# TimZaman/dotaclient

Hardware: NVIDIA H100
Metric: optimizer_steps_per_sec (higher is better)
Workload: dtype f32

## Files before the change

dotaclient_b200/csrc/encoder.cu:

```cuda
#include "dc_common.cuh"
#include "unit_basic.cuh"

namespace {

constexpr int kC = 128;
constexpr int kIn = kUnitFeatures;
constexpr int kWarps = 8;
constexpr int kThreadsE = kWarps * 32;
constexpr int kMaxUnits = 40;

__global__ void unit_basic_bwd_reduce_kernel(const float *__restrict__ partial, int nblocks, float *__restrict__ dw_b,
                                             float *__restrict__ db_b, int accumulate) {
    const int i = blockIdx.x * blockDim.x + threadIdx.x;
    if (i >= kC * (kIn + 1)) return;
    float s = 0.f;
    for (int b = 0; b < nblocks; ++b) s += partial[(size_t)b * kC * (kIn + 1) + i];
    const int o = i / (kIn + 1), k = i % (kIn + 1);
    float *dst = k < kIn ? dw_b + o * kIn + k : db_b + o;
    *dst = accumulate ? *dst + s : s;
}

constexpr int kEnvIn = 3;
__global__ void __launch_bounds__(kThreadsE) env_fwd_kernel(const float *__restrict__ env, const float *__restrict__ w_e,
                                                            const float *__restrict__ b_e, float *__restrict__ out, int ld,
                                                            int64_t N) {
    const int lane = threadIdx.x & 31, warp = threadIdx.x >> 5;
    float w[4][kEnvIn], b[4];
#pragma unroll
    for (int c = 0; c < 4; ++c) {
        b[c] = b_e[lane * 4 + c];
#pragma unroll
        for (int k = 0; k < kEnvIn; ++k) w[c][k] = w_e[(lane * 4 + c) * kEnvIn + k];
    }
    const int64_t rows_per_iter = (int64_t)gridDim.x * kWarps * 32;
    for (int64_t base = ((int64_t)blockIdx.x * kWarps + warp) * 32; base < N; base += rows_per_iter) {
        const int nrows = (int)min((int64_t)32, N - base);
        float e[kEnvIn];
#pragma unroll
        for (int k = 0; k < kEnvIn; ++k) e[k] = lane < nrows ? env[(base + lane) * kEnvIn + k] : 0.f;
        for (int r = 0; r < nrows; ++r) {
            float a[4] = {b[0], b[1], b[2], b[3]};
#pragma unroll
            for (int k = 0; k < kEnvIn; ++k) {
                const float u = __shfl_sync(0xffffffffu, e[k], r);
#pragma unroll
                for (int c = 0; c < 4; ++c) a[c] = fmaf(u, w[c][k], a[c]);
            }
            *reinterpret_cast<float4 *>(out + (base + r) * ld + lane * 4) =
                make_float4(fmaxf(a[0], 0.f), fmaxf(a[1], 0.f), fmaxf(a[2], 0.f), fmaxf(a[3], 0.f));
        }
    }
}

__global__ void __launch_bounds__(kThreadsE) env_bwd_kernel(const float *__restrict__ d_out, const float *__restrict__ out, int ld,
                                                            const float *__restrict__ env, int64_t N,
                                                            float *__restrict__ partial) {
    __shared__ float s_red[kC][kEnvIn + 1];
    const int lane = threadIdx.x & 31, warp = threadIdx.x >> 5;
    float acc[4][kEnvIn + 1];
#pragma unroll
    for (int c = 0; c < 4; ++c)
#pragma unroll
        for (int k = 0; k <= kEnvIn; ++k) acc[c][k] = 0.f;
    const int64_t rows_per_iter = (int64_t)gridDim.x * kWarps * 32;
    for (int64_t base = ((int64_t)blockIdx.x * kWarps + warp) * 32; base < N; base += rows_per_iter) {
        const int nrows = (int)min((int64_t)32, N - base);
        float e[kEnvIn];
#pragma unroll
        for (int k = 0; k < kEnvIn; ++k) e[k] = lane < nrows ? env[(base + lane) * kEnvIn + k] : 0.f;
        for (int r0 = 0; r0 < nrows; r0 += 8) {
            float4 g4[8], y4[8];
#pragma unroll
            for (int j = 0; j < 8; ++j) {
                const int r = min(r0 + j, nrows - 1);
                g4[j] = __ldg(reinterpret_cast<const float4 *>(d_out + (base + r) * ld) + lane);
                y4[j] = __ldg(reinterpret_cast<const float4 *>(out + (base + r) * ld) + lane);
            }
#pragma unroll
            for (int j = 0; j < 8; ++j) {
                const bool live = r0 + j < nrows;
                const float g[4] = {live && y4[j].x > 0.f ? g4[j].x : 0.f, live && y4[j].y > 0.f ? g4[j].y : 0.f,
                                    live && y4[j].z > 0.f ? g4[j].z : 0.f, live && y4[j].w > 0.f ? g4[j].w : 0.f};
#pragma unroll
                for (int k = 0; k < kEnvIn; ++k) {
                    const float u = __shfl_sync(0xffffffffu, e[k], min(r0 + j, 31));
#pragma unroll
                    for (int c = 0; c < 4; ++c) acc[c][k] = fmaf(g[c], u, acc[c][k]);
                }
#pragma unroll
                for (int c = 0; c < 4; ++c) acc[c][kEnvIn] += g[c];
            }
        }
    }
    for (int w = 0; w < kWarps; ++w) {
        if (warp == w) {
#pragma unroll
            for (int c = 0; c < 4; ++c)
#pragma unroll
                for (int k = 0; k <= kEnvIn; ++k) {
                    float *dst = &s_red[lane * 4 + c][k];
                    *dst = (w == 0 ? 0.f : *dst) + acc[c][k];
                }
        }
        __syncthreads();
    }
    for (int i = threadIdx.x; i < kC * (kEnvIn + 1); i += kThreadsE)
        partial[(size_t)blockIdx.x * kC * (kEnvIn + 1) + i] = (&s_red[0][0])[i];
}

__global__ void __launch_bounds__(256) env_bwd_reduce_kernel(const float *__restrict__ partial, int nblocks, float *__restrict__ dw_e,
                                                             float *__restrict__ db_e) {
    __shared__ float sh[8][32];
    const int x = threadIdx.x & 31, y = threadIdx.x >> 5;
    const int i = blockIdx.x * 32 + x;
    float s = 0.f;
    if (i < kC * (kEnvIn + 1))
        for (int b = y; b < nblocks; b += 8) s += partial[(size_t)b * kC * (kEnvIn + 1) + i];
    sh[y][x] = s;
    __syncthreads();
    if (y == 0 && i < kC * (kEnvIn + 1)) {
        float t = 0.f;
#pragma unroll
        for (int r = 0; r < 8; ++r) t += sh[r][x];
        const int o = i / (kEnvIn + 1), k = i % (kEnvIn + 1);
        if (k < kEnvIn) dw_e[o * kEnvIn + k] = t; else db_e[o] = t;
    }
}

struct UnitPtrs { const float *p[6]; };
__host__ __device__ constexpr int group_units(int g) { return g == 1 ? 5 : (g == 2 || g == 3) ? 16 : 1; }
__host__ __device__ constexpr int group_offset(int g) { return g == 0 ? 0 : g == 1 ? 1 : g == 2 ? 6 : g == 3 ? 22 : g == 4 ? 38 : 39; }
constexpr int kTokenU4 = kMaxUnits * kIn / 4;

__device__ __forceinline__ void load_basic_weights(float (&w)[4][kIn], float (&b)[4], const float *__restrict__ w_b,
                                                   const float *__restrict__ b_b, int lane) {
#pragma unroll
    for (int c = 0; c < 4; ++c) {
        b[c] = __ldg(b_b + 4 * lane + c);
#pragma unroll
        for (int k = 0; k < kIn; ++k) w[c][k] = __ldg(w_b + (4 * lane + c) * kIn + k);
    }
}

__device__ __forceinline__ void stage_token_units(float4 *su, const UnitPtrs &units, int64_t n, int lane) {
#pragma unroll
    for (int g = 0; g < 6; ++g) {
        const int cnt = 3 * group_units(g);
        const float4 *src = reinterpret_cast<const float4 *>(units.p[g]) + n * cnt;
        for (int j = lane; j < cnt; j += 32) su[3 * group_offset(g) + j] = __ldg(src + j);
    }
}

__device__ __forceinline__ float4 basic_row(const float4 *row, const float (&w)[4][kIn], const float (&b)[4]) {
    const float4 u0 = row[0], u1 = row[1], u2 = row[2];
    const float u[kIn] = {u0.x, u0.y, u0.z, u0.w, u1.x, u1.y, u1.z, u1.w, u2.x, u2.y, u2.z, u2.w};
    return make_float4(dc_unit_basic(u, w[0], b[0]), dc_unit_basic(u, w[1], b[1]), dc_unit_basic(u, w[2], b[2]),
                       dc_unit_basic(u, w[3], b[3]));
}

__global__ void __launch_bounds__(kThreadsE) target_unit_q_fwd_kernel(const float *__restrict__ q, int ld_q, UnitPtrs units,
                                                                      const float *__restrict__ w_b, const float *__restrict__ b_b,
                                                                      float *__restrict__ logits, int64_t N) {
    __shared__ float4 s_u[kWarps][kTokenU4];
    const int lane = threadIdx.x & 31, warp = threadIdx.x >> 5;
    float w[4][kIn], b[4];
    load_basic_weights(w, b, w_b, b_b, lane);
    float4 *su = s_u[warp];
    for (int64_t n = (int64_t)blockIdx.x * kWarps + warp; n < N; n += (int64_t)gridDim.x * kWarps) {
        const float *qrow = q + n * ld_q;
        __syncwarp();
        stage_token_units(su, units, n, lane);
        __syncwarp();
        float mine = 0.f, mine_hi = 0.f;
#pragma unroll
        for (int g = 0; g < 6; ++g) {
            const float4 a = __ldg(reinterpret_cast<const float4 *>(qrow + g * kC) + lane);
            const float c = __ldg(qrow + 6 * kC + g);
            const int nu = group_units(g), off = group_offset(g);
            for (int u = 0; u < nu; ++u) {
                const float4 v = basic_row(su + 3 * (off + u), w, b);
                float d = v.x * a.x + v.y * a.y + v.z * a.z + v.w * a.w;
                d = dc_warp_sum(d) + c;
                const int o = off + u;
                if (o < 32) { if (lane == o) mine = d; } else { if (lane == o - 32) mine_hi = d; }
            }
        }
        logits[n * kMaxUnits + lane] = mine;
        if (lane < kMaxUnits - 32) logits[n * kMaxUnits + 32 + lane] = mine_hi;
    }
}

__global__ void __launch_bounds__(kThreadsE) target_unit_q_bwd_kernel(const float *__restrict__ dlogits, UnitPtrs units,
                                                                      const float *__restrict__ w_b, const float *__restrict__ b_b,
                                                                      float *__restrict__ s, int ld_s, int64_t N) {
    __shared__ float4 s_u[kWarps][kTokenU4];
    const int lane = threadIdx.x & 31, warp = threadIdx.x >> 5;
    float w[4][kIn], b[4];
    load_basic_weights(w, b, w_b, b_b, lane);
    float4 *su = s_u[warp];
    const float4 zero = make_float4(0.f, 0.f, 0.f, 0.f);
    for (int64_t n = (int64_t)blockIdx.x * kWarps + warp; n < N; n += (int64_t)gridDim.x * kWarps) {
        const float g_lo = dlogits[n * kMaxUnits + lane];
        const float g_hi = lane < kMaxUnits - 32 ? dlogits[n * kMaxUnits + 32 + lane] : 0.f;
        const bool any = __any_sync(0xffffffffu, g_lo != 0.f || g_hi != 0.f);
        float4 *srow = reinterpret_cast<float4 *>(s + n * ld_s) + lane;
        if (!any) {
#pragma unroll
            for (int g = 0; g < 7; ++g) srow[g * (kC / 4)] = zero;
            continue;
        }
        __syncwarp();
        stage_token_units(su, units, n, lane);
        __syncwarp();
        float sig[6];
#pragma unroll
        for (int g = 0; g < 6; ++g) {
            const int nu = group_units(g), off = group_offset(g);
            float4 acc = zero;
            float sg = 0.f;
            for (int u = 0; u < nu; ++u) {
                const int o = off + u;
                const float gv = __shfl_sync(0xffffffffu, o < 32 ? g_lo : g_hi, o & 31);
                const float4 v = basic_row(su + 3 * o, w, b);
                acc.x = fmaf(gv, v.x, acc.x); acc.y = fmaf(gv, v.y, acc.y); acc.z = fmaf(gv, v.z, acc.z); acc.w = fmaf(gv, v.w, acc.w);
                sg += gv;
            }
            srow[g * (kC / 4)] = acc;
            sig[g] = sg;
        }
        float4 tail = zero;
        if (lane == 0) tail = make_float4(sig[0], sig[1], sig[2], sig[3]);
        if (lane == 1) tail = make_float4(sig[4], sig[5], 0.f, 0.f);
        srow[6 * (kC / 4)] = tail;
    }
}

static unsigned head_grid(int per_sm, int64_t N) {
    const int64_t want = (N + kWarps - 1) / kWarps, cap = (int64_t)(per_sm < 1 ? 1 : per_sm) * dc_sm_count();
    return (unsigned)(want < cap ? want : cap);
}

static int unit_ptrs(const float *const units[6], UnitPtrs *up, const char *who) {
    DC_REQUIRE(units != nullptr, DC_EINVAL, "%s: units is NULL", who);
    for (int g = 0; g < 6; ++g) {
        DC_REQUIRE(units[g] && ((uintptr_t)units[g] & 15) == 0, DC_EINVAL, "%s: units[%d] null / not 16-byte aligned", who, g);
        up->p[g] = units[g];
    }
    return DC_OK;
}

}

extern "C" size_t dc_unit_basic_bwd_workspace_bytes(void) { return (size_t)4 * 1024 * kC * (kIn + 1) * sizeof(float); }

int dc_unit_basic_reduce(const float *partial, int nblocks, float *dw_b, float *db_b, int accumulate, cudaStream_t st) {
    unit_basic_bwd_reduce_kernel<<<(kC * (kIn + 1) + 255) / 256, 256, 0, st>>>(partial, nblocks, dw_b, db_b, accumulate);
    DC_LAUNCH_OK();
    return DC_OK;
}

extern "C" int dc_env_fwd(const float *env, const float *w_e, const float *b_e, float *out, int ld_out, int64_t N,
                          dc_stream_t stream) {
    DC_REQUIRE(env && w_e && b_e && out && N > 0 && ld_out >= kC && ld_out % 4 == 0 && ((uintptr_t)out & 15) == 0, DC_EINVAL,
               "dc_env_fwd: bad arguments");
    env_fwd_kernel<<<4 * dc_sm_count(), kThreadsE, 0, dc_cu_stream(stream)>>>(env, w_e, b_e, out, ld_out, N);
    DC_LAUNCH_OK();
    return DC_OK;
}

extern "C" size_t dc_env_bwd_workspace_bytes(void) { return (size_t)1024 * kC * (kEnvIn + 1) * sizeof(float); }

extern "C" int dc_env_bwd(const float *d_out, const float *out, int ld, const float *env, float *dw_e, float *db_e, int64_t N,
                          void *workspace, dc_stream_t stream) {
    DC_REQUIRE(d_out && out && env && dw_e && db_e && workspace && N > 0 && ld >= kC && ld % 4 == 0, DC_EINVAL,
               "dc_env_bwd: bad arguments");
    DC_REQUIRE((((uintptr_t)d_out | (uintptr_t)out) & 15) == 0, DC_EINVAL, "dc_env_bwd: inputs must be 16-byte aligned");
    cudaStream_t st = dc_cu_stream(stream);
    float *partial = reinterpret_cast<float *>(workspace);
    const int blocks = 2 * dc_sm_count();
    env_bwd_kernel<<<blocks, kThreadsE, 0, st>>>(d_out, out, ld, env, N, partial);
    DC_LAUNCH_OK();
    env_bwd_reduce_kernel<<<(kC * (kEnvIn + 1) + 31) / 32, 256, 0, st>>>(partial, blocks, dw_e, db_e);
    DC_LAUNCH_OK();
    return DC_OK;
}

extern "C" int dc_target_unit_q_fwd(const float *q, int ld_q, const float *const units[6], const float *w_b, const float *b_b,
                                    float *logits, int64_t N, dc_stream_t stream) {
    DC_REQUIRE(q && w_b && b_b && logits && N > 0 && ld_q >= 7 * kC && ld_q % 4 == 0, DC_EINVAL, "dc_target_unit_q_fwd: bad arguments");
    UnitPtrs up;
    const int rc = unit_ptrs(units, &up, "dc_target_unit_q_fwd");
    if (rc != DC_OK) return rc;
    DC_REQUIRE(((uintptr_t)q & 15) == 0, DC_EINVAL, "dc_target_unit_q_fwd: alignment");
    int per_sm = 0;
    DC_CUDA(cudaOccupancyMaxActiveBlocksPerMultiprocessor(&per_sm, target_unit_q_fwd_kernel, kThreadsE, 0));
    target_unit_q_fwd_kernel<<<head_grid(per_sm, N), kThreadsE, 0, dc_cu_stream(stream)>>>(q, ld_q, up, w_b, b_b, logits, N);
    DC_LAUNCH_OK();
    return DC_OK;
}

extern "C" int dc_target_unit_q_bwd(const float *dlogits, const float *const units[6], const float *w_b, const float *b_b, float *s,
                                    int ld_s, int64_t N, dc_stream_t stream) {
    DC_REQUIRE(dlogits && w_b && b_b && s && N > 0 && ld_s >= 7 * kC && ld_s % 4 == 0, DC_EINVAL, "dc_target_unit_q_bwd: bad arguments");
    UnitPtrs up;
    const int rc = unit_ptrs(units, &up, "dc_target_unit_q_bwd");
    if (rc != DC_OK) return rc;
    DC_REQUIRE(((uintptr_t)s & 15) == 0, DC_EINVAL, "dc_target_unit_q_bwd: alignment");
    int per_sm = 0;
    DC_CUDA(cudaOccupancyMaxActiveBlocksPerMultiprocessor(&per_sm, target_unit_q_bwd_kernel, kThreadsE, 0));
    target_unit_q_bwd_kernel<<<head_grid(per_sm, N), kThreadsE, 0, dc_cu_stream(stream)>>>(dlogits, up, w_b, b_b, s, ld_s, N);
    DC_LAUNCH_OK();
    return DC_OK;
}
```

Measured before the change: 79.06.

## Double-buffer target-unit head forward with cp.async and transposed warp reductions

Rewrites the target-unit Q forward kernel to prefetch the next token's unit features and q row into shared memory with cp.async double buffering, overlapping loads with compute. It replaces the per-unit full warp-sum reductions with a batched transpose-reduce across 8 units at a time, cutting shuffle count. Block size drops to 4 warps to fit the larger shared slots. This adds shared memory pressure and register use from the fully unrolled 40-unit loop.

```diff
diff --git a/dotaclient_b200/csrc/encoder.cu b/dotaclient_b200/csrc/encoder.cu
--- a/dotaclient_b200/csrc/encoder.cu
+++ b/dotaclient_b200/csrc/encoder.cu
@@ -158,36 +158,102 @@
                        dc_unit_basic(u, w[3], b[3]));
 }
 
-__global__ void __launch_bounds__(kThreadsE) target_unit_q_fwd_kernel(const float *__restrict__ q, int ld_q, UnitPtrs units,
-                                                                      const float *__restrict__ w_b, const float *__restrict__ b_b,
-                                                                      float *__restrict__ logits, int64_t N) {
-    __shared__ float4 s_u[kWarps][kTokenU4];
+constexpr int kHeadWarps = 4;
+constexpr int kHeadThreads = kHeadWarps * 32;
+constexpr int kHeadQ4 = (6 * kC + 8) / 4;
+constexpr int kHeadSlot4 = kTokenU4 + kHeadQ4;
+
+__device__ __forceinline__ int unit_group(int o) { return o < 1 ? 0 : o < 6 ? 1 : o < 22 ? 2 : o < 38 ? 3 : o < 39 ? 4 : 5; }
+
+__device__ __forceinline__ void cp_async16(uint32_t dst, const void *src) {
+    asm volatile("cp.async.cg.shared.global [%0], [%1], 16;" ::"r"(dst), "l"(src) : "memory");
+}
+
+constexpr int kHeadU4PerLane = (kTokenU4 + 31) / 32;
+struct HeadUnitPieces {
+    const float4 *src[kHeadU4PerLane];
+    int cnt[kHeadU4PerLane];
+};
+__device__ __forceinline__ HeadUnitPieces head_unit_pieces(const UnitPtrs &units, int lane) {
+    HeadUnitPieces pc;
+#pragma unroll
+    for (int i = 0; i < kHeadU4PerLane; ++i) {
+        const int j = min(lane + 32 * i, kTokenU4 - 1), g = unit_group(j / 3);
+        const float *p = units.p[0];
+#pragma unroll
+        for (int h = 1; h < 6; ++h) p = g == h ? units.p[h] : p;
+        pc.src[i] = reinterpret_cast<const float4 *>(p) + (j - 3 * group_offset(g));
+        pc.cnt[i] = 3 * group_units(g);
+    }
+    return pc;
+}
+
+__device__ __forceinline__ void head_copy_token(float4 *slot, const float *__restrict__ q, int ld_q, const HeadUnitPieces &pc,
+                                                int64_t n, int lane) {
+    const uint32_t dst = (uint32_t)__cvta_generic_to_shared(slot);
+#pragma unroll
+    for (int i = 0; i < kHeadU4PerLane; ++i)
+        if (lane + 32 * i < kTokenU4) cp_async16(dst + 16 * (lane + 32 * i), pc.src[i] + n * pc.cnt[i]);
+    const float4 *qsrc = reinterpret_cast<const float4 *>(q + n * ld_q);
+#pragma unroll
+    for (int i = 0; i < (kHeadQ4 + 31) / 32; ++i)
+        if (lane + 32 * i < kHeadQ4) cp_async16(dst + 16 * (kTokenU4 + lane + 32 * i), qsrc + lane + 32 * i);
+}
+
+__device__ __forceinline__ void transpose_reduce8(float (&p)[8], int lane) {
+#pragma unroll
+    for (int k = 16, h = 4; k >= 4; k >>= 1, h >>= 1) {
+        const bool upper = lane & k;
+#pragma unroll
+        for (int i = 0; i < h; ++i) {
+            const float keep = upper ? p[i + h] : p[i], send = upper ? p[i] : p[i + h];
+            p[i] = keep + __shfl_xor_sync(0xffffffffu, send, k);
+        }
+    }
+    p[0] += __shfl_xor_sync(0xffffffffu, p[0], 2);
+    p[0] += __shfl_xor_sync(0xffffffffu, p[0], 1);
+}
+
+__global__ void __launch_bounds__(kHeadThreads) target_unit_q_fwd_kernel(const float *__restrict__ q, int ld_q, UnitPtrs units,
+                                                                         const float *__restrict__ w_b, const float *__restrict__ b_b,
+                                                                         float *__restrict__ logits, int64_t N) {
+    __shared__ float4 s_slot[kHeadWarps][2][kHeadSlot4];
     const int lane = threadIdx.x & 31, warp = threadIdx.x >> 5;
     float w[4][kIn], b[4];
     load_basic_weights(w, b, w_b, b_b, lane);
-    float4 *su = s_u[warp];
-    for (int64_t n = (int64_t)blockIdx.x * kWarps + warp; n < N; n += (int64_t)gridDim.x * kWarps) {
-        const float *qrow = q + n * ld_q;
+    const HeadUnitPieces pieces = head_unit_pieces(units, lane);
+    const int64_t stride = (int64_t)gridDim.x * kHeadWarps;
+    int64_t n = (int64_t)blockIdx.x * kHeadWarps + warp;
+    if (n < N) head_copy_token(s_slot[warp][0], q, ld_q, pieces, n, lane);
+    asm volatile("cp.async.commit_group;" ::: "memory");
+    const int row_lo = 8 * (lane & 3) + (lane >> 2), row_hi = 32 + (lane >> 2);
+    for (int it = 0; n < N; n += stride, ++it) {
         __syncwarp();
-        stage_token_units(su, units, n, lane);
+        head_copy_token(s_slot[warp][(it + 1) & 1], q, ld_q, pieces, n + stride < N ? n + stride : n, lane);
+        asm volatile("cp.async.commit_group;" ::: "memory");
+        asm volatile("cp.async.wait_group 1;" ::: "memory");
         __syncwarp();
-        float mine = 0.f, mine_hi = 0.f;
-#pragma unroll
-        for (int g = 0; g < 6; ++g) {
-            const float4 a = __ldg(reinterpret_cast<const float4 *>(qrow + g * kC) + lane);
-            const float c = __ldg(qrow + 6 * kC + g);
-            const int nu = group_units(g), off = group_offset(g);
-            for (int u = 0; u < nu; ++u) {
-                const float4 v = basic_row(su + 3 * (off + u), w, b);
-                float d = v.x * a.x + v.y * a.y + v.z * a.z + v.w * a.w;
-                d = dc_warp_sum(d) + c;
-                const int o = off + u;
-                if (o < 32) { if (lane == o) mine = d; } else { if (lane == o - 32) mine_hi = d; }
-            }
-        }
-        logits[n * kMaxUnits + lane] = mine;
-        if (lane < kMaxUnits - 32) logits[n * kMaxUnits + 32 + lane] = mine_hi;
-    }
+        const float4 *su = s_slot[warp][it & 1];
+        const float4 *qs = su + kTokenU4;
+        float4 a_g[6];
+#pragma unroll
+        for (int g = 0; g < 6; ++g) a_g[g] = qs[g * (kC / 4) + lane];
+        float mine = 0.f, mine_hi = 0.f, p[8];
+#pragma unroll
+        for (int o = 0; o < kMaxUnits; ++o) {
+            const float4 v = basic_row(su + 3 * o, w, b);
+            const float4 &a = a_g[unit_group(o)];
+            p[o & 7] = v.x * a.x + v.y * a.y + v.z * a.z + v.w * a.w;
+            if ((o & 7) == 7) {
+                transpose_reduce8(p, lane);
+                if (o < 32) { if ((lane & 3) == (o >> 3)) mine = p[0]; } else mine_hi = p[0];
+            }
+        }
+        const float *qf = reinterpret_cast<const float *>(qs);
+        logits[n * kMaxUnits + row_lo] = mine + qf[6 * kC + unit_group(row_lo)];
+        if ((lane & 3) == 0) logits[n * kMaxUnits + row_hi] = mine_hi + qf[6 * kC + unit_group(row_hi)];
+    }
+    asm volatile("cp.async.wait_all;" ::: "memory");
 }
 
 __global__ void __launch_bounds__(kThreadsE) target_unit_q_bwd_kernel(const float *__restrict__ dlogits, UnitPtrs units,
@@ -235,8 +301,8 @@
     }
 }
 
-static unsigned head_grid(int per_sm, int64_t N) {
-    const int64_t want = (N + kWarps - 1) / kWarps, cap = (int64_t)(per_sm < 1 ? 1 : per_sm) * dc_sm_count();
+static unsigned head_grid(int per_sm, int warps, int64_t N) {
+    const int64_t want = (N + warps - 1) / warps, cap = (int64_t)(per_sm < 1 ? 1 : per_sm) * dc_sm_count();
     return (unsigned)(want < cap ? want : cap);
 }
 
@@ -293,8 +359,9 @@
     if (rc != DC_OK) return rc;
     DC_REQUIRE(((uintptr_t)q & 15) == 0, DC_EINVAL, "dc_target_unit_q_fwd: alignment");
     int per_sm = 0;
-    DC_CUDA(cudaOccupancyMaxActiveBlocksPerMultiprocessor(&per_sm, target_unit_q_fwd_kernel, kThreadsE, 0));
-    target_unit_q_fwd_kernel<<<head_grid(per_sm, N), kThreadsE, 0, dc_cu_stream(stream)>>>(q, ld_q, up, w_b, b_b, logits, N);
+    DC_CUDA(cudaOccupancyMaxActiveBlocksPerMultiprocessor(&per_sm, target_unit_q_fwd_kernel, kHeadThreads, 0));
+    target_unit_q_fwd_kernel<<<head_grid(per_sm, kHeadWarps, N), kHeadThreads, 0, dc_cu_stream(stream)>>>(q, ld_q, up, w_b, b_b,
+                                                                                                          logits, N);
     DC_LAUNCH_OK();
     return DC_OK;
 }
@@ -308,7 +375,7 @@
     DC_REQUIRE(((uintptr_t)s & 15) == 0, DC_EINVAL, "dc_target_unit_q_bwd: alignment");
     int per_sm = 0;
     DC_CUDA(cudaOccupancyMaxActiveBlocksPerMultiprocessor(&per_sm, target_unit_q_bwd_kernel, kThreadsE, 0));
-    target_unit_q_bwd_kernel<<<head_grid(per_sm, N), kThreadsE, 0, dc_cu_stream(stream)>>>(dlogits, up, w_b, b_b, s, ld_s, N);
-    DC_LAUNCH_OK();
-    return DC_OK;
-}
+    target_unit_q_bwd_kernel<<<head_grid(per_sm, kWarps, N), kThreadsE, 0, dc_cu_stream(stream)>>>(dlogits, up, w_b, b_b, s, ld_s, N);
+    DC_LAUNCH_OK();
+    return DC_OK;
+}
```

Result: faster. 80.77, median of 6 (+2.2%).
